# Mathiasb17/Nereus

Measured on AMD Instinct MI355X. Metric: particle-steps/sec, SESPH dam-break, higher is better.
Workload: dtype f32

## Files before the change

### nereus_amd/csrc/nrs_kernels_tiled.h

```cpp
#pragma once
#include "nrs_kernels_ref.h"
#include "nrs_kernels_slab.h"
#include <type_traits>

namespace nrs {

constexpr int HIT_CAP = 20;
constexpr uint32_t HIT_INDEX = (1u << 27) - 1;
constexpr int HIT_TAG_SHIFT = 27;

struct CutThresholds { float lenLtIr, r2LeH2; };

#ifndef FORCES_LISTS_MIN_WAVES
#define FORCES_LISTS_MIN_WAVES 7
#endif
#ifndef FORCES_PACKED_MIN_WAVES
#define FORCES_PACKED_MIN_WAVES 5
#endif
#ifndef FORCES_PACKED_MIN_WAVES_UNFUSED
#define FORCES_PACKED_MIN_WAVES_UNFUSED 4
#endif
NRS_DEV float bcast_lane(float v, int srcLane) { return __int_as_float(__builtin_amdgcn_readlane(__float_as_int(v), srcLane)); }
NRS_DEV double bcast_lane(double v, int srcLane)
{
    const long long b = __double_as_longlong(v);
    const int lo = __builtin_amdgcn_readlane((int)(b & 0xffffffffll), srcLane), hi = __builtin_amdgcn_readlane((int)(b >> 32), srcLane);
    return __longlong_as_double(((long long)hi << 32) | (long long)(unsigned int)lo);
}
#ifndef NRS_DBG_LDS_PAD
#define NRS_DBG_LDS_PAD 0
#endif
#ifndef NRS_DBG_LDS_PAD_F
#define NRS_DBG_LDS_PAD_F 0
#endif
#ifndef QP_WALK
#define QP_WALK 4
#endif
#ifndef QP_PRE
#define QP_PRE 2
#endif
constexpr int SCAN_CAP = 21;
NRS_DEV int mad24(int a, int b, int c)
{
    int d;
    asm("v_mad_i32_i24 %0, %1, %2, %3" : "=v"(d) : "v"(a), "v"(b), "v"(c));
    return d;
}
constexpr int SCAN_BATCH = 4;

struct HitCounts { int nf, nb; bool over; bool anyB; };
constexpr uint32_t GATHER_STRIDE = 2u;
template <typename R> struct PrePair { R prq, mrho; };

template <typename R> struct Sweep {
    typedef typename Vec4T<R>::type T4;
    static NRS_DEV T4 at32(const T4 *__restrict__ base, uint32_t idx)
    {
        const uint32_t off = idx * (uint32_t)sizeof(T4);
        return *reinterpret_cast<const T4 *>(reinterpret_cast<const char *>(base) + off);
    }

    template <bool HAS_B, int BFILT, int W, bool FWIDE = false>
    static NRS_DEV HitCounts scan(const Params<R> &P, const GridView<R> &G, const CutThresholds thr,
                                  const T4 *__restrict__ sPos, uint32_t self, V3<R> p, uint32_t (*lst)[W])
    {
        const I3 gp = calcGridPos<R>(P, p);
        const uint32_t mx = P.gridSize[0] - 1, my = P.gridSize[1] - 1, mz = P.gridSize[2] - 1;
        const uint32_t cx = grid_x<R>(P, gp.x);
        const uint32_t x0 = (cx - 1u) & mx, x2 = (cx + 1u) & mx;
        const bool contiguous = (cx >= 1u) && (cx + 1u <= mx);
        const float tF = FWIDE ? thr.r2LeH2 : thr.lenLtIr;
        const float tB = BFILT == 2 ? INFINITY : (BFILT == 1 ? thr.r2LeH2 : thr.lenLtIr);
        const uint32_t tid = threadIdx.x;
        int nf = 0, nb = 0;
        bool over = false, anyB = false;

        auto sweepFluid = [&](uint32_t a, uint32_t b, uint32_t m1, uint32_t m2, uint32_t tag0) {
            const uint32_t nT = run_ok<R>(G, a, b) ? b - a : 0u;
            for (uint32_t base = 0; base < nT; base += SCAN_BATCH) {
                T4 c[SCAN_BATCH];
#pragma unroll
                for (int u = 0; u < SCAN_BATCH; ++u) c[u] = at32(sPos, a + min(base + (uint32_t)u, nT - 1u));
#pragma unroll
                for (int u = 0; u < SCAN_BATCH; ++u) {
                    const uint32_t q = base + (uint32_t)u;
                    const uint32_t j = a + q;
                    const V3<R> d = p - xyz<R>(c[u]);
                    const bool hit = (q < nT) & (j != self) & (dot(d, d) < tF);
                    if (hit) {
                        uint32_t tag = tag0 + (((m1 != CELL_EMPTY) & (j >= m1)) ? 1u : 0u);
                        if ((m2 != CELL_EMPTY) & (j >= m2)) tag = tag0 + 2u;
                        if (nf + nb < HIT_CAP) lst[nf][tid] = j | (tag << HIT_TAG_SHIFT); else over = true;
                        ++nf;
                    }
                }
            }
        };

        for (int z = -1; z <= 1; z++) {
            const uint32_t cz = (uint32_t)(gp.z + z) & mz;
            const uint32_t plane = umul24(umul24(cz, P.gridSize[1]), P.gridSize[0]);
            uint32_t st[3][3], en[3][3], hrow[3];
            uint32_t bmask = 0;
#pragma unroll
            for (int y = 0; y < 3; ++y) {
                const uint32_t cy = (uint32_t)(gp.y + y - 1) & my;
                hrow[y] = plane + umul24(cy, P.gridSize[0]);
                const uint32_t h[3] = {hrow[y] + x0, hrow[y] + cx, hrow[y] + x2};
#pragma unroll
                for (int c = 0; c < 3; ++c) {
                    st[y][c] = G.cellStart[h[c]];
                    en[y][c] = G.cellEnd[h[c]];
                    if (HAS_B) bmask |= (G.bCellStart[h[c]] != CELL_EMPTY) ? (1u << (y * 3 + c)) : 0u;
                }
            }
#pragma unroll
            for (int y = 0; y < 3; ++y) {
                const uint32_t tag0 = (uint32_t)((z + 1) * 9 + y * 3);
                const uint32_t s0 = st[y][0], s1 = st[y][1], s2 = st[y][2];
                if (contiguous) {
                    uint32_t lo = (s0 != CELL_EMPTY) ? s0 : ((s1 != CELL_EMPTY) ? s1 : s2);
                    uint32_t hi = (s2 != CELL_EMPTY) ? en[y][2] : ((s1 != CELL_EMPTY) ? en[y][1] : en[y][0]);
                    if (lo == CELL_EMPTY) lo = hi = 0;
                    sweepFluid(lo, hi, s1, s2, tag0);
                } else {
#pragma unroll
                    for (int c = 0; c < 3; ++c)
                        if (st[y][c] != CELL_EMPTY) sweepFluid(st[y][c], en[y][c], CELL_EMPTY, CELL_EMPTY, tag0 + (uint32_t)c);
                }
            }
            if (HAS_B) {
                anyB = anyB || bmask != 0u;
                if (BFILT == 2) bmask = 0u;
                while (bmask) {
                    const int bit = __builtin_ctz(bmask);
                    bmask &= bmask - 1u;
                    const int y = bit / 3, c = bit - y * 3;
                    const uint32_t cy = (uint32_t)(gp.y + y - 1) & my;
                    const uint32_t hc = plane + umul24(cy, P.gridSize[0]) + (c == 0 ? x0 : (c == 1 ? cx : x2));
                    const uint32_t a = G.bCellStart[hc], nT = G.bCellEnd[hc] - a;
                    const uint32_t tag = (uint32_t)((z + 1) * 9 + bit);
                    for (uint32_t base = 0; base < nT; base += 4) {
                        T4 cb[4];
#pragma unroll
                        for (int u = 0; u < 4; ++u) cb[u] = G.sB[a + min(base + (uint32_t)u, nT - 1u)];
#pragma unroll
                        for (int u = 0; u < 4; ++u) {
                            const uint32_t q = base + (uint32_t)u;
                            const V3<R> d = p - xyz<R>(cb[u]);
                            if ((q < nT) & (dot(d, d) < tB)) {
                                if (nf + nb < HIT_CAP) lst[HIT_CAP - 1 - nb][tid] = (a + q) | (tag << HIT_TAG_SHIFT); else over = true;
                                ++nb;
                            }
                        }
                    }
                }
            }
        }
        HitCounts hc;
        const bool finite = (fabs(p.x) < (R)INFINITY) & (fabs(p.y) < (R)INFINITY) & (fabs(p.z) < (R)INFINITY);
        hc.nf = nf; hc.nb = nb; hc.over = over | !finite; hc.anyB = anyB;
        return hc;
    }

    static constexpr int QSLOTS = 16 / sizeof(qword_t);
    struct __attribute__((packed, aligned(sizeof(qword_t)))) Q2 { uint32_t v[4]; };
    static NRS_DEV Q2 ldq(const qword_t *__restrict__ qpos, uint32_t idx)
    {
        return *reinterpret_cast<const Q2 *>(reinterpret_cast<const char *>(qpos) + idx * (uint32_t)sizeof(qword_t));
    }
    template <int W>
    static NRS_DEV HitCounts scan_compact(const Params<R> &P, const GridView<R> &G, V3<R> p, uint32_t (*lst)[W])
    {
        const I3 gp = calcGridPos<R>(P, p);
        const uint32_t mx = P.gridSize[0] - 1, my = P.gridSize[1] - 1, mz = P.gridSize[2] - 1;
        const uint32_t cx = grid_x<R>(P, gp.x);
        const uint32_t x0 = (cx - 1u) & mx, x2 = (cx + 1u) & mx;
        const bool contiguous = (cx >= 1u) && (cx + 1u <= mx);
        float tx, ty, tz;
        quantize_t<R>(G.qc, p, tx, ty, tz);
        const bool far = !((fabsf(tx) < QP_FAR) & (fabsf(ty) < QP_FAR) & (fabsf(tz) < QP_FAR));
        const uint32_t Qi = pack_quanta(tx, ty, tz) | QP_GUARD;
        const uint32_t qT = G.qT;
        const qword_t *__restrict__ qpos = G.qpos;
        const uint32_t col = threadIdx.x * 4u, rowBytes = (uint32_t)W * 4u, capOff = col + (uint32_t)(SCAN_CAP + 1) * rowBytes;
        uint32_t cur = col;
        char *const lbase = reinterpret_cast<char *>(&lst[0][0]);

        auto test2 = [&](const Q2 &c, uint32_t aTag, uint32_t base, uint32_t nT) {
#pragma unroll
            for (int u = 0; u < QSLOTS; ++u) {
                if ((u & 1) == 0) cur = min(cur, capOff);
                const uint32_t t = Qi - c.v[u];
                const int dx = ((int)(t << 22)) >> 22, dy = ((int)(t << 11)) >> 22, dz = ((int)t) >> 22;
                const uint32_t d2 = (uint32_t)mad24(dz, dz, mad24(dy, dy, __mul24(dx, dx)));
                const uint32_t q = base + (uint32_t)u;
                const bool hit = (d2 < qT) & (q < nT);
                *reinterpret_cast<uint32_t *>(lbase + cur) = aTag + q;
                cur += hit ? rowBytes : 0u;
            }
        };
        auto sweepRun = [&](uint32_t aTag, uint32_t nT, uint32_t from) {
            for (uint32_t base = from; base < nT; base += QSLOTS) test2(ldq(qpos, (aTag & HIT_INDEX) + base), aTag, base, nT);
        };

        for (int z = -1; z <= 1; z++) {
            const uint32_t cz = (uint32_t)(gp.z + z) & mz;
            const uint32_t plane = umul24(umul24(cz, P.gridSize[1]), P.gridSize[0]);
            uint32_t st[3][3], en[3][3];
#pragma unroll
            for (int y = 0; y < 3; ++y) {
                const uint32_t cy = (uint32_t)(gp.y + y - 1) & my;
                const uint32_t hrow = plane + umul24(cy, P.gridSize[0]);
                const uint32_t h[3] = {hrow + x0, hrow + cx, hrow + x2};
#pragma unroll
                for (int c = 0; c < 3; ++c) {
                    const uint32_t off = h[c] * 4u;
                    st[y][c] = *reinterpret_cast<const uint32_t *>(reinterpret_cast<const char *>(G.cellStart) + off);
                    en[y][c] = *reinterpret_cast<const uint32_t *>(reinterpret_cast<const char *>(G.cellEnd) + off);
                }
            }
            if (contiguous) {
                uint32_t lo[3], nT[3];
#pragma unroll
                for (int y = 0; y < 3; ++y) {
                    const uint32_t s0 = st[y][0], s1 = st[y][1], s2 = st[y][2];
                    uint32_t a = (s0 != CELL_EMPTY) ? s0 : ((s1 != CELL_EMPTY) ? s1 : s2);
                    uint32_t b = (s2 != CELL_EMPTY) ? en[y][2] : ((s1 != CELL_EMPTY) ? en[y][1] : en[y][0]);
                    if (a == CELL_EMPTY) a = b = 0;
                    const bool ok = run_ok<R>(G, a, b);
                    lo[y] = ok ? a : 0u;
                    nT[y] = ok ? b - a : 0u;
                }
                Q2 c[3][QP_PRE];
#pragma unroll
                for (int y = 0; y < 3; ++y)
#pragma unroll
                    for (int k = 0; k < QP_PRE; ++k) c[y][k] = ldq(qpos, lo[y] + min((uint32_t)(QSLOTS * k), nT[y]));
#pragma unroll
                for (int y = 0; y < 3; ++y) {
                    const uint32_t aTag = lo[y] | ((uint32_t)((z + 1) * 9 + y * 3) << HIT_TAG_SHIFT);
#pragma unroll
                    for (int k = 0; k < QP_PRE; ++k)
                        if (k == 0 || nT[y] > (uint32_t)(QSLOTS * k))
                            test2(c[y][k], aTag, (uint32_t)(QSLOTS * k), nT[y]);
                    sweepRun(aTag, nT[y], (uint32_t)(QSLOTS * QP_PRE));
                }
            } else {
#pragma unroll
                for (int y = 0; y < 3; ++y)
#pragma unroll
                    for (int c = 0; c < 3; ++c)
                        if (st[y][c] != CELL_EMPTY && run_ok<R>(G, st[y][c], en[y][c]))
                            sweepRun(st[y][c] | ((uint32_t)((z + 1) * 9 + y * 3) << HIT_TAG_SHIFT), en[y][c] - st[y][c], 0u);
            }
        }
        const uint32_t nf = (cur - col) / rowBytes;
        HitCounts hc;
        hc.nf = (int)nf; hc.nb = 0; hc.over = far || nf > (uint32_t)SCAN_CAP; hc.anyB = false;
        return hc;
    }
};

struct HitMerge {
    const uint32_t *base;
    uint32_t stride;
    int nf, nb, kf, kb;
    uint32_t headF, headB;
    NRS_DEV HitMerge(const uint32_t *b, uint32_t st, HitCounts hc) : base(b), stride(st), nf(hc.nf), nb(hc.nb), kf(0), kb(0)
    {
        headF = nf > 0 ? base[0] : 0xffffffffu;
        headB = nb > 0 ? base[(uint32_t)(HIT_CAP - 1) * stride] : 0xffffffffu;
    }
    NRS_DEV int last_boundary() const { return kb - 1; }
    NRS_DEV bool next(uint32_t &index, bool &boundary, uint32_t &key)
    {
        if (kf >= nf && kb >= nb) return false;
        const uint32_t tf = headF >> HIT_TAG_SHIFT, tb = headB >> HIT_TAG_SHIFT;
        boundary = tb < tf;
        const uint32_t e = boundary ? headB : headF;
        if (boundary) {
            ++kb;
            headB = kb < nb ? base[(uint32_t)(HIT_CAP - 1 - kb) * stride] : 0xffffffffu;
        } else {
            ++kf;
            headF = kf < nf ? base[(uint32_t)kf * stride] : 0xffffffffu;
        }
        index = e & HIT_INDEX;
        key = (e >> HIT_TAG_SHIFT) * 2u + (boundary ? 1u : 0u);
        return true;
    }
};

template <typename R, int KSET, bool HAS_B, bool STRICT = false, bool BOUNDARY_BY_CELL = false>
NRS_DEV R density_from_hits(const Params<R> &P, const GridView<R> &G, const typename Vec4T<R>::type *__restrict__ sPos,
                            V3<R> p, const uint32_t *lbase, uint32_t lstride, HitCounts hc, uint32_t self = 0xffffffffu)
{
    const R ir = P.interactionRadius, kp = P.kpoly, pm = P.particleMass, rd = P.restDensity;
    R d = (R)0.0;
    d += pm * W_dens<R, KSET>(mk3<R>(0, 0, 0), ir, kp);
    if (BOUNDARY_BY_CELL) {
        const I3 gp = calcGridPos<R>(P, p);
        int k = 0;
        uint32_t head = hc.nf > 0 ? lbase[0] : 0xffffffffu;
        uint32_t c = 0;
        for (int z = -1; z <= 1; z++)
            for (int y = -1; y <= 1; y++)
                for (int x = -1; x <= 1; x++, c++) {
                    if ((head >> HIT_TAG_SHIFT) == c) {
                        R part = (R)0.0;
                        do {
                            const uint32_t j = head & HIT_INDEX;
                            const V3<R> r = p - xyz<R>(sPos[j]);
                            if (!STRICT || ((j != self) && (length(r) < ir))) part += (pm * W_dens<R, KSET>(r, ir, kp));
                            ++k;
                            head = k < hc.nf ? lbase[(uint32_t)k * lstride] : 0xffffffffu;
                        } while ((head >> HIT_TAG_SHIFT) == c);
                        d += part;
                    }
                    if (hc.anyB) {
                        const uint32_t h = calcGridHash<R>(P, gp.x + x, gp.y + y, gp.z + z);
                        const uint32_t sB = G.bCellStart[h];
                        if (sB != CELL_EMPTY) {
                            const uint32_t eB = G.bCellEnd[h];
                            R part = (R)0.0;
                            for (uint32_t j = sB; j < eB; ++j) {
                                const typename Vec4T<R>::type b = G.sB[j];
                                const V3<R> r = p - xyz<R>(b);
                                if (length(r) < ir) part += ((rd * b.w) * W_dens<R, KSET>(r, ir, kp));
                            }
                            d += part;
                        }
                    }
                }
        return d;
    }
    R part = (R)0.0;
    uint32_t prevKey = 0xffffffffu;
    HitMerge it(lbase, lstride, hc);
    uint32_t j, key;
    bool isB;
    while (it.next(j, isB, key)) {
        if (key != prevKey) { d += part; part = (R)0.0; prevKey = key; }
        if (HAS_B && isB) {
            const typename Vec4T<R>::type b = G.sB[j];
            const V3<R> r = p - xyz<R>(b);
            if (length(r) < ir) {
                const R psi = rd * b.w;
                part += (psi * W_dens<R, KSET>(r, ir, kp));
            }
        } else {
            const V3<R> r = p - xyz<R>(sPos[j]);
            if (!STRICT || ((j != self) && (length(r) < ir))) part += (pm * W_dens<R, KSET>(r, ir, kp));
        }
    }
    d += part;
    return d;
}

template <typename R, int KSET, bool STRICT, bool INRANGE = false>
NRS_DEV R density_from_superset(const Params<R> &P, const typename Vec4T<R>::type *__restrict__ sPos, V3<R> p, uint32_t (*lst)[BLOCK],
                                int &nf, float tKeep, uint32_t self)
{
    const uint32_t tid = threadIdx.x;
    const R ir = P.interactionRadius, kp = P.kpoly, pm = P.particleMass;
    const uint32_t mx = P.gridSize[0] - 1;
    const int gxi = (int)floor((p.x - P.worldOrigin[0]) / P.cellSize[0]);
    float yCell = 0.f;
    if constexpr (INRANGE) yCell = rcp_refined((float)P.cellSize[0]);
    R d = (R)0.0;
    d += pm * W_dens<R, KSET>(mk3<R>(0, 0, 0), ir, kp);
    R part = (R)0.0;
    uint32_t prevTag = 0xffffffffu;
    int w = 0;
    for (int k0 = 0; k0 < nf; k0 += QP_WALK) {
        uint32_t e[QP_WALK];
        V3<R> q[QP_WALK];
#pragma unroll
        for (int u = 0; u < QP_WALK; ++u) e[u] = lst[min(k0 + u, nf - 1)][tid];
#pragma unroll
        for (int u = 0; u < QP_WALK; ++u) q[u] = xyz<R>(sPos[e[u] & HIT_INDEX]);
#pragma unroll
        for (int u = 0; u < QP_WALK; ++u) {
            const V3<R> r = p - q[u];
            const uint32_t j = e[u] & HIT_INDEX;
            const float d2 = dot(r, r);
            if ((k0 + u < nf) && (d2 < tKeep) && (STRICT || j != self)) {
                int gxj;
                if constexpr (INRANGE) gxj = (int)floor(div_steps((float)(q[u].x - P.worldOrigin[0]), (float)P.cellSize[0], yCell));
                else gxj = (int)floor((q[u].x - P.worldOrigin[0]) / P.cellSize[0]);
                const uint32_t tag = (e[u] >> HIT_TAG_SHIFT) + (((uint32_t)(gxj - gxi) + 1u) & mx);
                lst[min(w, HIT_CAP - 1)][tid] = j | (tag << HIT_TAG_SHIFT);
                ++w;
                if (tag != prevTag) { d += part; part = (R)0.0; prevTag = tag; }
                if constexpr (INRANGE) {
                    const float len = d2 >= 0x1p-96f ? sqrt_inrange(d2) : sqrt_rn(d2);
                    if (!STRICT || ((j != self) && (len < ir))) {
                        const float r2 = len * len, h2 = ir * ir;
                        part += (pm * (r2 > h2 ? 0.0f : kp * cube_via_double<float>(h2 - r2)));
                    }
                } else {
                    if (!STRICT || ((j != self) && (length(r) < ir))) part += (pm * W_dens<R, KSET>(r, ir, kp));
                }
            }
        }
    }
    d += part;
    nf = w;
    return d;
}
template <typename R> NRS_DEV bool density_inrange_ok(const Params<R> &P, V3<R> p)
{
    if constexpr (!std::is_same<R, float>::value) return false;
    else {
        const float cs = P.cellSize[0], wo = fabsf(P.worldOrigin[0]);
        if (!(cs >= 0x1p-20f && cs <= 0x1p10f && wo <= 0x1p60f)) return false;
        if (wo >= 0x1p-60f) return true;
        return __all(fabsf(p.x - P.worldOrigin[0]) >= 4.0f * cs) != 0;
    }
}

template <typename R, int KSET> struct BoundaryTerms { V3<R> bound, pres, visc; };
template <typename R, int KSET>
NRS_DEV BoundaryTerms<R, KSET> boundary_terms(const Params<R> &P, V3<R> pos1, V3<R> vel1, R dens, R pres, typename Vec4T<R>::type bq)
{
    const R pm = P.particleMass, ir = P.interactionRadius;
    const R epsilon = (R)0.01;
    const R beta = P.beta, rd = P.restDensity;
    const R psi = (rd * bq.w);
    const V3<R> rij = pos1 - xyz<R>(bq);
    const V3<R> vij = vel1;
    R kernel;
    V3<R> grad;
    if (KSET == KS_MONAGHAN) {
        kernel = Wmonaghan<R>(rij, ir);
        grad = Wmonaghan_grad<R>(rij, ir);
    } else {
        kernel = Wdefault<R>(rij, ir, P.kpoly);
        grad = Wdefault_grad<R>(rij, ir, P.kpoly_grad);
    }
    BoundaryTerms<R, KSET> T;
    T.bound = (beta * psi * rij * kernel);
    T.pres = (-pm * psi * (pres / (dens * dens)) * grad);
    const R nuWall = (P.viscosity * ir * P.soundSpeed) / (dens * dens);
    const R approach = (R)fmax((double)dot(vij, rij), 0.0);
    const R normSq = dot(rij / length(rij), rij / length(rij)) + epsilon * ir * ir;
    const R friction = -nuWall * (approach / normSq);
    T.visc = (pm * psi * friction * grad);
    return T;
}

NRS_DEV f2 div2(f2 a, f2 b) { return pair2(a.x / b.x, a.y / b.y); }
struct InRange { float yVisc; uint32_t loBits, spanBits; bool constantsOk; };
NRS_DEV InRange in_range_setup(const Params<float> &P)
{
    InRange G;
    const float h = P.interactionRadius, h2 = h * h, kvd = fabsf(P.kvisc_denum);
    G.constantsOk = h >= 0x1p-10f && h <= 0x1p10f && kvd >= 0x1p-40f && kvd <= 0x1p40f;
    G.yVisc = rcp_refined(P.kvisc_denum);
    G.loBits = __float_as_uint(h2 * 0x1p-16f);
    G.spanBits = __float_as_uint(h2 * 2.0f) - G.loBits;
    return G;
}

struct PairTerms2 { V3x2 pres, visc, surf; };
template <bool SURF, bool INRANGE>
NRS_DEV PairTerms2 fluid_terms2_muller(const Params<float> &P, V3<float> pos1, V3<float> vel1, float own, float c0, float wAtDiameter, float diameter2,
                                       float4 pa, float4 pb, float4 va, float4 vb, PrePair<float> qa, PrePair<float> qb, const InRange &G, bool &bad)
{
    const float ir = P.interactionRadius, m2 = P.particleMass;
    float rxa = pos1.x - pa.x, rxb = pos1.x - pb.x, rya = pos1.y - pa.y, ryb = pos1.y - pb.y, rza = pos1.z - pa.z, rzb = pos1.z - pb.z;
    float vxa = vel1.x - va.x, vxb = vel1.x - vb.x, vya = vel1.y - va.y, vyb = vel1.y - vb.y, vza = vel1.z - va.z, vzb = vel1.z - vb.z;
    asm volatile("" : "+v"(rxa), "+v"(rxb), "+v"(rya), "+v"(ryb), "+v"(rza), "+v"(rzb));
    asm volatile("" : "+v"(vxa), "+v"(vxb), "+v"(vya), "+v"(vyb), "+v"(vza), "+v"(vzb));
    const V3x2 r = {pair2(rxa, rxb), pair2(rya, ryb), pair2(rza, rzb)};
    const V3x2 v = {pair2(vxa, vxb), pair2(vya, vyb), pair2(vza, vzb)};
    const f2 d2 = dot2(r, r);
    f2 len;
    if (INRANGE) {
        bad = bad || (__float_as_uint(d2.x) - G.loBits >= G.spanBits) || (__float_as_uint(d2.y) - G.loBits >= G.spanBits);
        len = sqrt_inrange2(d2);
    } else {
        len = pair2(sqrt_rn(d2.x), sqrt_rn(d2.y));
    }
    const f2 r2 = len * len;
    const float h2 = ir * ir;
    const bool outA = r2.x > h2, outB = r2.y > h2;
    const f2 hm = splat2(ir) - len;
    const f2 c = hm * hm;
    V3x2 gs;
    const f2 t3 = splat2(3.0f) * len;
    const f2 l3 = splat2(2.0f) * len * len * len;
    f2 cv;
    if (INRANGE) {
        const f2 y = rcp_refined2(len);
        gs.x = splat2(P.kpress_grad) * div_steps2(r.x, len, y) * c;
        gs.y = splat2(P.kpress_grad) * div_steps2(r.y, len, y) * c;
        gs.z = splat2(P.kpress_grad) * div_steps2(r.z, len, y) * c;
        cv = -div_steps2(t3, splat2(P.kvisc_denum), splat2(G.yVisc)) + splat2(2.0f / h2) - div_steps2(splat2(ir), l3, rcp_refined2(l3));
    } else {
        gs.x = splat2(P.kpress_grad) * div2(r.x, len) * c;
        gs.y = splat2(P.kpress_grad) * div2(r.y, len) * c;
        gs.z = splat2(P.kpress_grad) * div2(r.z, len) * c;
        cv = -div2(t3, splat2(P.kvisc_denum)) + splat2(2.0f / h2) - div2(splat2(ir), l3);
    }
    V3x2 gv = {splat2(P.kvisc_grad) * r.x * cv, splat2(P.kvisc_grad) * r.y * cv, splat2(P.kvisc_grad) * r.z * cv};
    const f2 hr = splat2(h2) - r2;
    f2 kern = splat2(P.kpoly) * pair2(cube_via_double<float>(hr.x), cube_via_double<float>(hr.y));
    if (outA) { gs.x.x = 0.f; gs.y.x = 0.f; gs.z.x = 0.f; gv.x.x = 0.f; gv.y.x = 0.f; gv.z.x = 0.f; kern.x = 0.f; }
    if (outB) { gs.x.y = 0.f; gs.y.y = 0.f; gs.z.y = 0.f; gv.x.y = 0.f; gv.y.y = 0.f; gv.z.y = 0.f; kern.y = 0.f; }
    PairTerms2 T;
    const f2 sp = splat2(m2) * (splat2(own) + pair2(qa.prq, qb.prq));
    T.pres.x = sp * gs.x; T.pres.y = sp * gs.y; T.pres.z = sp * gs.z;
    const f2 a = dot2(r, gv);
    const f2 b = d2 + splat2(0.01f * (ir * ir));
    const f2 q = div2(a, b);
    const f2 mr = pair2(qa.mrho, qb.mrho);
    T.visc.x = mr * v.x * q; T.visc.y = mr * v.y * q; T.visc.z = mr * v.z * q;
    if (SURF) {
        const f2 ks = pair2(d2.x > diameter2 ? kern.x : wAtDiameter, d2.y > diameter2 ? kern.y : wAtDiameter);
        const f2 z = splat2(0.f);
        T.surf.x = z - splat2(c0) * r.x * ks; T.surf.y = z - splat2(c0) * r.y * ks; T.surf.z = z - splat2(c0) * r.z * ks;
    }
    return T;
}

constexpr int LIST_BATCH = 4;
template <int NB = LIST_BATCH, typename GATHER, typename USE>
NRS_DEV void walk_fluid_batched(const uint32_t *col, uint32_t stride, int nf, GATHER &&gather, USE &&use)
{
    for (int k0 = 0; k0 < nf; k0 += NB) {
        uint32_t e[NB];
        decltype(gather(0u)) d[NB];
#pragma unroll
        for (int u = 0; u < NB; ++u) e[u] = col[(size_t)min(k0 + u, nf - 1) * stride];
#pragma unroll
        for (int u = 0; u < NB; ++u) d[u] = gather(e[u] & HIT_INDEX);
#pragma unroll
        for (int u = 0; u < NB; ++u)
            if (k0 + u < nf) use(e[u] & HIT_INDEX, e[u] >> HIT_TAG_SHIFT, d[u]);
    }
}

template <typename R, int KSET, bool SURF, bool HAS_B, bool STRICT = false, bool PAIRS = false, bool BOUNDARY_BY_CELL = false>
NRS_DEV ForceAcc<R> forces_from_hits(const Params<R> &P, const GridView<R> &G,
                                     const typename Vec4T<R>::type *__restrict__ sPos,
                                     const typename Vec4T<R>::type *__restrict__ sVel, const R *__restrict__ sDens,
                                     const R *__restrict__ sPres, V3<R> pos1, V3<R> vel1, R dens, R pres,
                                     const uint32_t *lbase, uint32_t lstride, HitCounts hc, uint32_t self = 0xffffffffu,
                                     const R *pre = nullptr, const typename Vec4T<R>::type *__restrict__ gpos = nullptr,
                                     const typename Vec4T<R>::type *__restrict__ gvel = nullptr, const uint32_t *__restrict__ lroot = nullptr,
                                     uint32_t lcol = 0u)
{
    ForceAcc<R> A;
    A.fpres = A.fvisc = A.fsurf = A.fbound = mk3<R>(0, 0, 0);
    const R pm = P.particleMass, m2 = P.particleMass, ir = P.interactionRadius, kp = P.kpoly;
    const R kappa = P.surfaceTension;
    const R kprg = P.kpress_grad, kvg = P.kvisc_grad, kvd = P.kvisc_denum;
    const R diameter = (R)(2.0 * P.particleRadius);
    const R diameter2 = diameter * diameter;
    const R rhoSqOwn = dens * dens;
    R wAtDiameter;
    if (KSET == KS_MONAGHAN) wAtDiameter = Wmonaghan<R>(mk3<R>(diameter, 0, 0), ir);
    else wAtDiameter = Wdefault<R>(mk3<R>(diameter, 0, 0), ir, kp);
    const R epsilon = (R)0.01;
    const R beta = P.beta, rd = P.restDensity;
    auto boundaryHit = [&](const BoundaryTerms<R, KSET> &T) {
        A.fbound = A.fbound + T.bound;
        A.fpres = A.fpres + T.pres;
        A.fvisc = A.fvisc - T.visc;
    };
    auto fluidHit = [&](uint32_t j) {
        V3<R> rij, vij;
        R pOverRhoSqNb, mOverRhoNb;
        if (PAIRS) {
            const typename Vec4T<R>::type a = gpos[GATHER_STRIDE * j], b = gvel[GATHER_STRIDE * j];
            rij = pos1 - xyz<R>(a);
            if (STRICT && ((j == self) || !(length(rij) < ir))) return;
            vij = vel1 - xyz<R>(b);
            pOverRhoSqNb = a.w; mOverRhoNb = b.w;
        } else {
            rij = pos1 - xyz<R>(sPos[j]);
            if (STRICT && ((j == self) || !(length(rij) < ir))) return;
            const R rhoNb = sDens[j];
            const R pNb = sPres[j];
            const R rhoSqNb = rhoNb * rhoNb;
            pOverRhoSqNb = pNb / rhoSqNb; mOverRhoNb = m2 / rhoNb;
            vij = vel1 - xyz<R>(sVel[j]);
        }
        V3<R> gradSpiky, gradVisc;
        R kernel;
        if (KSET == KS_MONAGHAN) {
            gradSpiky = Wmonaghan_grad<R>(rij, ir);
            gradVisc = gradSpiky;
            kernel = Wmonaghan<R>(rij, ir);
        } else {
            gradSpiky = Wpressure_grad<R>(rij, ir, kprg);
            gradVisc = Wviscosity_grad<R>(rij, ir, kvg, kvd);
            kernel = Wdefault<R>(rij, ir, kp);
        }
        A.fpres = A.fpres + (m2 * (pres / rhoSqOwn + pOverRhoSqNb) * gradSpiky);
        const R a = dot(rij, gradVisc);
        const R b = dot(rij, rij) + 0.01f * (ir * ir);
        A.fvisc = A.fvisc + (mOverRhoNb * vij * (a / b));
        if (SURF) {
            V3<R> ai = mk3<R>(0, 0, 0);
            const R r2 = dot(rij, rij);
            if (r2 > diameter2) ai = ai - (kappa / pm * pm * rij * kernel);
            else ai = ai - (kappa / pm * pm * rij * wAtDiameter);
            A.fsurf = A.fsurf + ai;
        }
    };
    if (BOUNDARY_BY_CELL) {
        const I3 gp = calcGridPos<R>(P, pos1);
        int k = 0;
        uint32_t head = hc.nf > 0 ? lbase[0] : 0xffffffffu;
        uint32_t c = 0;
        for (int z = -1; z <= 1; z++)
            for (int y = -1; y <= 1; y++)
                for (int x = -1; x <= 1; x++, c++) {
                    while ((head >> HIT_TAG_SHIFT) == c) {
                        fluidHit(head & HIT_INDEX);
                        ++k;
                        head = k < hc.nf ? lbase[(uint32_t)k * lstride] : 0xffffffffu;
                    }
                    if (hc.anyB) {
                        const uint32_t h = calcGridHash<R>(P, gp.x + x, gp.y + y, gp.z + z);
                        const uint32_t sB = G.bCellStart[h];
                        if (sB != CELL_EMPTY) {
                            const uint32_t eB = G.bCellEnd[h];
                            for (uint32_t j = sB; j < eB; ++j) boundaryHit(boundary_terms<R, KSET>(P, pos1, vel1, dens, pres, G.sB[j]));
                        }
                    }
                }
        return A;
    }
    if constexpr (!HAS_B && !STRICT && PAIRS && KSET == KS_MULLER && std::is_same<R, float>::value) {
        const int nf = hc.nf;
        const float own = pres / rhoSqOwn, c0 = kappa / pm * pm;
        auto walk = [&](auto inRange, const InRange &IG, bool &bad) {
            ForceAcc<R> S;
            S.fpres = S.fvisc = S.fsurf = S.fbound = mk3<R>(0, 0, 0);
            auto entry = [&](int k) { return lroot[(size_t)k * lstride + lcol]; };
            uint32_t e0 = nf > 0 ? entry(0) : 0u, e1 = nf > 1 ? entry(1) : e0;
            for (int k = 0; k < nf; k += 2) {
                const uint32_t j0 = e0 & HIT_INDEX, j1 = e1 & HIT_INDEX;
                const bool two = k + 1 < nf;
                const uint32_t n0 = k + 2 < nf ? entry(k + 2) : 0u;
                const uint32_t n1 = k + 3 < nf ? entry(k + 3) : n0;
                const float4 pa = gpos[GATHER_STRIDE * j0], pb = gpos[GATHER_STRIDE * j1], va = gvel[GATHER_STRIDE * j0], vb = gvel[GATHER_STRIDE * j1];
                const PairTerms2 T = fluid_terms2_muller<SURF, decltype(inRange)::value>(P, pos1, vel1, own, c0, wAtDiameter, diameter2, pa, pb, va, vb,
                                                                                        PrePair<float>{pa.w, va.w}, PrePair<float>{pb.w, vb.w}, IG, bad);
                S.fpres = S.fpres + mk3<R>(T.pres.x.x, T.pres.y.x, T.pres.z.x);
                S.fvisc = S.fvisc + mk3<R>(T.visc.x.x, T.visc.y.x, T.visc.z.x);
                if (SURF) S.fsurf = S.fsurf + mk3<R>(T.surf.x.x, T.surf.y.x, T.surf.z.x);
                if (two) {
                    S.fpres = S.fpres + mk3<R>(T.pres.x.y, T.pres.y.y, T.pres.z.y);
                    S.fvisc = S.fvisc + mk3<R>(T.visc.x.y, T.visc.y.y, T.visc.z.y);
                    if (SURF) S.fsurf = S.fsurf + mk3<R>(T.surf.x.y, T.surf.y.y, T.surf.z.y);
                }
                e0 = n0; e1 = n1;
            }
            return S;
        };
        const InRange IG = in_range_setup(P);
        const bool ownerOk = fminf(fminf(fabsf(pos1.x), fabsf(pos1.y)), fabsf(pos1.z)) >= 0x1p-66f;
        bool again = true;
        if (IG.constantsOk && __all(ownerOk)) {
            again = false;
            A = walk(std::true_type{}, IG, again);
        }
        if (again) A = walk(std::false_type{}, IG, again);
        return A;
    }
    HitMerge it(lbase, lstride, hc);
    uint32_t j, key;
    bool isB;
    while (it.next(j, isB, key)) {
        if (HAS_B && isB) {
            BoundaryTerms<R, KSET> T;
            if (pre) {
                const R *t = pre + (size_t)it.last_boundary() * 9;
                T.bound = mk3<R>(t[0], t[1], t[2]); T.pres = mk3<R>(t[3], t[4], t[5]); T.visc = mk3<R>(t[6], t[7], t[8]);
            } else {
                T = boundary_terms<R, KSET>(P, pos1, vel1, dens, pres, G.sB[j]);
            }
            boundaryHit(T);
        } else {
            fluidHit(j);
        }
    }
    return A;
}

NRS_DEV uint32_t xcd_tile(uint32_t b, uint32_t nb)
{
    const uint32_t per = nb >> 3;
    return (b < (per << 3)) ? (b & 7u) * per + (b >> 3) : b;
}

struct FastPair { float pr, invRho; };
struct HitBuffer {
    uint32_t *hits; uint32_t *counts; uint32_t stride;
    void *gpos = nullptr, *gvel = nullptr;
    const void *svel = nullptr;
    FastPair *fast = nullptr;
};
template <typename R> NRS_DEV typename Vec4T<R>::type own_sorted_velocity(const HitBuffer &hb, uint32_t i)
{
    return reinterpret_cast<const typename Vec4T<R>::type *>(hb.svel)[i];
}
template <typename R>
NRS_DEV void publish_gather_records(const Params<R> &P, const HitBuffer &hb, uint32_t i, V3<R> p, typename Vec4T<R>::type v, R d, R pr)
{
    typedef typename Vec4T<R>::type T4;
    reinterpret_cast<T4 *>(hb.gpos)[GATHER_STRIDE * i] = mk4<R>(p, pr / (d * d));
    reinterpret_cast<T4 *>(hb.gvel)[GATHER_STRIDE * i] = mk4<R>(xyz<R>(v), P.particleMass / d);
}
NRS_DEV uint32_t pack_counts(HitCounts hc)
{
    return (uint32_t)hc.nf | ((uint32_t)hc.nb << 8) | (hc.over ? 1u << 16 : 0u) | (hc.anyB ? 1u << 17 : 0u);
}
constexpr uint32_t COUNTS_UNSTAGED = 1u << 18;
NRS_DEV HitCounts unpack_counts(uint32_t c)
{
    HitCounts hc;
    hc.nf = (int)(c & 0xffu); hc.nb = (int)((c >> 8) & 0xffu); hc.over = ((c >> 16) & 1u) != 0u;
    hc.anyB = ((c >> 17) & 1u) != 0u;
    return hc;
}

static __global__ __launch_bounds__(BLOCK) void k_hit_stats(const uint32_t *__restrict__ counts, unsigned long long *__restrict__ out, uint32_t n)
{
    unsigned long long over = 0, sum = 0, mx = 0, unst = 0;
    for (uint32_t i = blockIdx.x * BLOCK + threadIdx.x; i < n; i += gridDim.x * BLOCK) {
        const uint32_t c = counts[i];
        const HitCounts hc = unpack_counts(c);
        unst += (c & COUNTS_UNSTAGED) ? 1ull : 0ull;
        if (hc.over) { ++over; continue; }
        const unsigned long long k = (unsigned long long)(hc.nf + hc.nb);
        sum += k;
        mx = k > mx ? k : mx;
    }
    for (int d = 32; d >= 1; d >>= 1) {
        over += __shfl_down(over, d);
        sum += __shfl_down(sum, d);
        unst += __shfl_down(unst, d);
        const unsigned long long o = __shfl_down(mx, d);
        mx = o > mx ? o : mx;
    }
    if ((threadIdx.x & 63u) == 0) {
        atomicAdd(&out[0], over);
        atomicAdd(&out[1], sum);
        atomicMax(&out[2], mx);
        atomicAdd(&out[3], unst);
    }
}

constexpr uint32_t COUNTS_DEFERRED = 1u << 19;

NRS_DEV bool cell_near_boundary(const WallList &wl, uint32_t h) { return ((wl.nearBits[h >> 5] >> (h & 31u)) & 1u) != 0u; }

static __global__ __launch_bounds__(BLOCK) void k_wall_compact(WallList wl, const uint32_t *__restrict__ tileOffset, const uint32_t *__restrict__ groupPrefix,
                                                                 uint32_t groupSize, uint32_t *__restrict__ list, uint32_t n)
{
    __shared__ uint32_t waveCnt[BLOCK / 64];
    const uint32_t i = blockIdx.x * BLOCK + threadIdx.x, lane = threadIdx.x & 63u, wave = threadIdx.x >> 6;
    const unsigned long long m = wl.mask[i >> 6];
    const bool take = ((m >> lane) & 1ull) != 0ull;
    if (lane == 0) waveCnt[wave] = (uint32_t)__popcll(m);
    __syncthreads();
    if (!take) return;
    uint32_t before = (uint32_t)__popcll(m & ((1ull << lane) - 1ull));
    for (uint32_t w = 0; w < wave; ++w) before += waveCnt[w];
    list[groupPrefix[blockIdx.x / groupSize] + tileOffset[blockIdx.x] + before] = i;
}

template <typename R, int KSET, bool HAS_B, bool SHARE, bool WIDE>
NRS_DEV void density_tiled_particle(const Params<R> &P, const GridView<R> &G, const CutThresholds thr,
                                    const typename Vec4T<R>::type *__restrict__ sPos, R *__restrict__ dens, R *__restrict__ pres,
                                    const HitBuffer &hb, uint32_t i, V3<R> p, uint32_t (*lst)[BLOCK], uint32_t countFlags = 0u)
{
    const uint32_t tid = threadIdx.x;
    constexpr int BF = SHARE ? (KSET == KS_MULLER ? 1 : 2) : 0;
    constexpr bool COMPACT = !HAS_B && SHARE;
    HitCounts hc;
    R d;
    if constexpr (COMPACT) {
        hc = Sweep<R>::template scan_compact<BLOCK>(P, G, p, lst);
        if (hc.over) d = density_of<R, KSET, HAS_B>(P, G, sPos, i);
        else {
            constexpr bool CAN = KSET == KS_MULLER && std::is_same<R, float>::value;
            const float tKeep = WIDE ? thr.r2LeH2 : thr.lenLtIr;
            if (CAN && density_inrange_ok<R>(P, p)) d = density_from_superset<R, KSET, WIDE, CAN>(P, sPos, p, lst, hc.nf, tKeep, i);
            else d = density_from_superset<R, KSET, WIDE>(P, sPos, p, lst, hc.nf, tKeep, i);
            if (hc.nf > HIT_CAP) { hc.over = true; d = density_of<R, KSET, HAS_B>(P, G, sPos, i); }
        }
    } else {
        hc = Sweep<R>::template scan<HAS_B, BF, BLOCK, WIDE>(P, G, thr, sPos, WIDE ? 0xffffffffu : i, p, lst);
        if (hc.over) d = density_of<R, KSET, HAS_B>(P, G, sPos, i);
        else d = density_from_hits<R, KSET, HAS_B, WIDE, (HAS_B && BF == 2)>(P, G, sPos, p, &lst[0][tid], BLOCK, hc, i);
    }
    dens[i] = d;
    if (pres) {
        const R pr = tait_pressure<R>(P, d);
        pres[i] = pr;
        if (SHARE && hb.gpos) publish_gather_records<R>(P, hb, i, p, own_sorted_velocity<R>(hb, i), d, pr);
        if (SHARE && hb.fast) {
            const float inv = __builtin_amdgcn_rcpf((float)d);
            FastPair z;
            z.pr = (float)pr * inv * inv; z.invRho = inv;
            hb.fast[i] = z;
        }
    }
    if (SHARE) {
        hb.counts[i] = pack_counts(hc) | countFlags;
        if (!hc.over) {
            for (int k = 0; k < hc.nf; ++k) hb.hits[(size_t)k * hb.stride + i] = lst[k][tid];
            for (int k = 0; k < hc.nb; ++k) hb.hits[(size_t)(HIT_CAP - 1 - k) * hb.stride + i] = lst[HIT_CAP - 1 - k][tid];
        }
    }
}

#ifndef DENSITY_DEFER_MIN_WAVES
#define DENSITY_DEFER_MIN_WAVES 6
#endif
template <typename R, int KSET, bool HAS_B, bool SHARE, bool WIDE = false, bool DEFER = false>
__global__ __launch_bounds__(BLOCK, (((DEFER || (!HAS_B && SHARE)) && sizeof(R) == 4) ? DENSITY_DEFER_MIN_WAVES : 1)) void k_density_tiled(Params<R> P, GridView<R> G, CutThresholds thr,
                                                         const typename Vec4T<R>::type *__restrict__ sPos,
                                                         R *__restrict__ dens, R *__restrict__ pres, HitBuffer hb,
                                                         uint32_t n, WallList wl, uint32_t wallBlocks)
{
    constexpr int LIST_ROWS = (SHARE && (DEFER || !HAS_B)) ? SCAN_CAP + 3 : HIT_CAP;
    __shared__ uint32_t lst[LIST_ROWS][BLOCK];
    uint32_t block = blockIdx.x, blocks = gridDim.x;
    if (DEFER) {
        if (block < wallBlocks) {
            const uint32_t count = *wl.count;
            for (uint32_t t = block * BLOCK + threadIdx.x; t < count; t += wallBlocks * BLOCK) {
                const uint32_t i = wl.list[t];
                const V3<R> p = xyz<R>(sPos[i]);
                if (!slab_active<R>(P, G, p.x)) {
                    dens[i] = (R)0;
                    if (pres) pres[i] = (R)0;
                    hb.counts[i] = COUNTS_DEFERRED;
                    continue;
                }
                density_tiled_particle<R, KSET, true, SHARE, WIDE>(P, G, thr, sPos, dens, pres, hb, i, p, lst, COUNTS_DEFERRED);
            }
            return;
        }
        block -= wallBlocks; blocks -= wallBlocks;
    }
    const uint32_t i = xcd_tile(block, blocks) * BLOCK + threadIdx.x;
    if (i >= n) return;
    if (DEFER && ((wl.mask[i >> 6] >> (i & 63u)) & 1ull)) return;
    const V3<R> p = xyz<R>(sPos[i]);
    if (!slab_active<R>(P, G, p.x)) {
        dens[i] = (R)0;
        if (pres) pres[i] = (R)0;
        if (SHARE) hb.counts[i] = 0u;
        return;
    }
    density_tiled_particle<R, KSET, HAS_B, SHARE, WIDE>(P, G, thr, sPos, dens, pres, hb, i, p, lst);
}

template <typename R> struct FusedOut {
    typedef typename Vec4T<R>::type T4;
    T4 *newPos, *newVel;
    uint32_t *hash, *index;
    const uint32_t *prevHash;
    uint32_t *tileMovers;
    uint8_t *slabFlags;
    uint32_t *slabBlockCounts;
    uint32_t slabBlocks;
    uint32_t *tileDead;
    SlabCfg slab;
};

template <typename R, int KSET, bool SURF, bool HAS_B, bool FUSE>
NRS_DEV void forces_epilogue(const Params<R> &P, typename Vec4T<R>::type p4, typename Vec4T<R>::type v4, V3<R> f,
                             typename Vec4T<R>::type *__restrict__ forces, const FusedOut<R> &fo, uint32_t i)
{
    if (forces) forces[i] = mk4<R>(f, (R)0);
    if (FUSE) {
        const R dt = P.timestep, m1 = P.particleMass;
        const V3<R> pos1 = xyz<R>(p4), vel1 = xyz<R>(v4);
        const V3<R> accel = dt * f / m1;
        const V3<R> v = vel1 + accel;
        const V3<R> pn = pos1 + dt * v;
        fo.newPos[i] = mk4<R>(pn, p4.w);
        fo.newVel[i] = mk4<R>(v, v4.w);
        const I3 g = calcGridPos<R>(P, pn);
        const uint32_t h = calcGridHash<R>(P, g.x, g.y, g.z);
        uint32_t key = h;
        if (fo.slabFlags) {
            const uint32_t f = slab_flags<R>(P, fo.slab, mk4<R>(pn, p4.w));
            fo.slabFlags[i] = (uint8_t)f;
            if (!(f & (1u << ST_STAY))) {
                key = 0xffffffffu;
                atomicAdd(&fo.tileDead[i / BLOCK], 1u);
            } else if (h != fo.prevHash[i]) {
                atomicAdd(&fo.tileMovers[i / BLOCK], 1u);
            }
            if (f & ~(1u << ST_STAY))
                for (int s = 1; s < ST_COUNT; ++s)
                    if ((f >> s) & 1u) atomicAdd(&fo.slabBlockCounts[(uint32_t)s * fo.slabBlocks + i / SLAB_TILE], 1u);
        } else if (fo.tileMovers && h != fo.prevHash[i]) {
            atomicAdd(&fo.tileMovers[i / BLOCK], 1u);
        }
        fo.hash[i] = key;
        fo.index[i] = i;
    }
}

template <typename R, int KSET, bool SURF, bool HAS_B, bool FUSE>
__global__ __launch_bounds__(BLOCK) void k_forces_tiled(Params<R> P, GridView<R> G, CutThresholds thr,
                                                        const typename Vec4T<R>::type *__restrict__ sPos,
                                                        const typename Vec4T<R>::type *__restrict__ sVel,
                                                        const R *__restrict__ sDens, const R *__restrict__ sPres,
                                                        typename Vec4T<R>::type *__restrict__ forces, FusedOut<R> fo,
                                                        uint32_t n)
{
    typedef typename Vec4T<R>::type T4;
    __shared__ uint32_t lst[HIT_CAP][BLOCK];
    const uint32_t i = xcd_tile(blockIdx.x, gridDim.x) * BLOCK + threadIdx.x;
    if (i >= n) return;
    const uint32_t tid = threadIdx.x;
    const T4 p4 = sPos[i];
    const T4 v4 = sVel[i];
    const V3<R> pos1 = xyz<R>(p4), vel1 = xyz<R>(v4);
    V3<R> f = mk3<R>(0, 0, 0);
    if (slab_active<R>(P, G, pos1.x)) {
        const R dens = sDens[i], pres = sPres[i];
        constexpr int BF = (KSET == KS_MULLER ? 1 : 2);
        const HitCounts hc = Sweep<R>::template scan<HAS_B, BF, BLOCK>(P, G, thr, sPos, i, pos1, lst);
        ForceAcc<R> A;
        if (hc.over) A = gather_forces<R, KSET, SURF, HAS_B>(P, G, i, pos1, vel1, dens, pres, sPos, sVel, sDens, sPres);
        else A = forces_from_hits<R, KSET, SURF, HAS_B, false, false, (HAS_B && BF == 2)>(P, G, sPos, sVel, sDens, sPres, pos1, vel1, dens, pres, &lst[0][tid], BLOCK, hc);
        f = sesph_total_force<R>(P, A, dens);
    }
    forces_epilogue<R, KSET, SURF, HAS_B, FUSE>(P, p4, v4, f, forces, fo, i);
}

template <typename R, int KSET, bool SURF, bool HAS_B, bool FUSE>
NRS_DEV void forces_lists_particle(const Params<R> &P, const GridView<R> &G, const HitBuffer &hb,
                                   const typename Vec4T<R>::type *__restrict__ sPos, const typename Vec4T<R>::type *__restrict__ sVel,
                                   const R *__restrict__ sDens, const R *__restrict__ sPres, typename Vec4T<R>::type *__restrict__ forces,
                                   const FusedOut<R> &fo, uint32_t i, typename Vec4T<R>::type p4, typename Vec4T<R>::type v4,
                                   bool active, HitCounts hc)
{
    const V3<R> pos1 = xyz<R>(p4), vel1 = xyz<R>(v4);
    V3<R> f = mk3<R>(0, 0, 0);
    if (active) {
        const R dens = sDens[i], pres = sPres[i];
        ForceAcc<R> A;
        if (hc.over) A = gather_forces<R, KSET, SURF, HAS_B>(P, G, i, pos1, vel1, dens, pres, sPos, sVel, sDens, sPres);
        else
            A = forces_from_hits<R, KSET, SURF, HAS_B, false, true, (HAS_B && KSET == KS_MONAGHAN)>(P, G, sPos, sVel, sDens, sPres, pos1, vel1, dens, pres, hb.hits + i, hb.stride,
                                                                                     hc, 0xffffffffu, nullptr, reinterpret_cast<const typename Vec4T<R>::type *>(hb.gpos),
                                                                                     reinterpret_cast<const typename Vec4T<R>::type *>(hb.gvel), hb.hits, i);
        f = sesph_total_force<R>(P, A, dens);
    }
    forces_epilogue<R, KSET, SURF, HAS_B, FUSE>(P, p4, v4, f, forces, fo, i);
}

template <typename R, int KSET, bool SURF, bool HAS_B, bool FUSE, bool DEFER = false>
__global__ __launch_bounds__(BLOCK, (sizeof(R) == 4 ? ((KSET == KS_MULLER && !HAS_B) ? (FUSE ? FORCES_PACKED_MIN_WAVES : FORCES_PACKED_MIN_WAVES_UNFUSED) : FORCES_LISTS_MIN_WAVES) : 1)) void k_forces_lists(Params<R> P, GridView<R> G, HitBuffer hb,
                                                        const typename Vec4T<R>::type *__restrict__ sPos,
                                                        const typename Vec4T<R>::type *__restrict__ sVel,
                                                        const R *__restrict__ sDens, const R *__restrict__ sPres,
                                                        typename Vec4T<R>::type *__restrict__ forces, FusedOut<R> fo,
                                                        uint32_t n, WallList wl, uint32_t wallBlocks)
{
    typedef typename Vec4T<R>::type T4;
    uint32_t block = blockIdx.x, blocks = gridDim.x;
    if (DEFER) {
        if (block < wallBlocks) {
            const uint32_t count = *wl.count;
            for (uint32_t t = block * BLOCK + threadIdx.x; t < count; t += wallBlocks * BLOCK) {
                const uint32_t i = wl.list[t];
                const T4 p4 = sPos[i];
                const bool active = slab_active<R>(P, G, p4.x);
                forces_lists_particle<R, KSET, SURF, true, FUSE>(P, G, hb, sPos, sVel, sDens, sPres, forces, fo, i, p4, sVel[i], active,
                                                                 unpack_counts(active ? hb.counts[i] : 0u));
            }
            return;
        }
        block -= wallBlocks; blocks -= wallBlocks;
    }
    const uint32_t i = xcd_tile(block, blocks) * BLOCK + threadIdx.x;
    if (i >= n) return;
    const uint32_t c = hb.counts[i];
    if (DEFER && (c & COUNTS_DEFERRED)) return;
    const T4 p4 = sPos[i];
    const bool active = slab_active<R>(P, G, p4.x);
    forces_lists_particle<R, KSET, SURF, HAS_B, FUSE>(P, G, hb, sPos, sVel, sDens, sPres, forces, fo, i, p4, sVel[i], active,
                                                      unpack_counts(active ? c : 0u));
}

template <typename R>
__global__ __launch_bounds__(BLOCK) void k_mark_near_boundary(Params<R> P, const uint32_t *__restrict__ bHash, uint32_t nb, uint32_t *__restrict__ nearBits)
{
    const uint32_t i = blockIdx.x * BLOCK + threadIdx.x;
    if (i >= nb) return;
    const uint32_t h = bHash[i];
    if (i && bHash[i - 1] == h) return;
    const uint32_t gx = P.gridSize[0], gy = P.gridSize[1];
    const int x = (int)((h & (gx - 1)) + P.numBodies), y = (int)((h / gx) & (gy - 1)), z = (int)(h / (gx * gy));
    for (int dz = -1; dz <= 1; ++dz)
        for (int dy = -1; dy <= 1; ++dy)
            for (int dx = -1; dx <= 1; ++dx) {
                const uint32_t c = calcGridHash<R>(P, x + dx, y + dy, z + dz);
                atomicOr(&nearBits[c >> 5], 1u << (c & 31u));
            }
}

static inline bool is_pow2(uint32_t v) { return v && !(v & (v - 1)); }

template <typename R> static inline CutThresholds make_thresholds(const Params<R> &P)
{
    CutThresholds t;
    const R ir = P.interactionRadius;
    {
        float T = (float)(ir * ir);
        auto ge = [&](float x) { return !((R)sqrtf(x) < ir); };
        while (ge(T) && T > 0.0f) T = nextafterf(T, 0.0f);
        while (!ge(T)) T = nextafterf(T, INFINITY);
        t.lenLtIr = T;
    }
    {
        const R h2 = ir * ir;
        float T = (float)h2;
        auto gt = [&](float x) { float l = sqrtf(x); R r2 = l * l; return r2 > h2; };
        while (gt(T) && T > 0.0f) T = nextafterf(T, 0.0f);
        while (!gt(T)) T = nextafterf(T, INFINITY);
        t.r2LeH2 = T;
    }
    return t;
}

static inline uint32_t wall_blocks(uint32_t interiorBlocks) { return std::min<uint32_t>(1024u, std::max<uint32_t>(1u, interiorBlocks / 16u)); }

template <typename R, int KSET, bool HAS_B>
static inline void launch_density_tiled(hipStream_t stream, const Params<R> &P, const GridView<R> &G, const HitBuffer *share,
                                        const typename Vec4T<R>::type *sPos, R *dens, R *pres, uint32_t n, const WallList *wall = nullptr)
{
    const CutThresholds thr = make_thresholds<R>(P);
    const dim3 g((n + BLOCK - 1) / BLOCK), b(BLOCK);
    const HitBuffer hb = share ? *share : HitBuffer{};
    constexpr unsigned pad = NRS_DBG_LDS_PAD;
    if (share) {
        if (HAS_B && wall) {
            const uint32_t wb = wall_blocks(g.x);
            hipLaunchKernelGGL((k_density_tiled<R, KSET, false, true, false, true>), dim3(g.x + wb), b, pad, stream, P, G, thr, sPos, dens, pres, hb, n,
                               *wall, wb);
        } else {
            hipLaunchKernelGGL((k_density_tiled<R, KSET, HAS_B, true>), g, b, pad, stream, P, G, thr, sPos, dens, pres, hb, n, WallList{}, 0u);
        }
    } else {
        hipLaunchKernelGGL((k_density_tiled<R, KSET, HAS_B, false>), g, b, 0, stream, P, G, thr, sPos, dens, pres, hb, n, WallList{}, 0u);
    }
}
template <typename R, int KSET, bool HAS_B>
static inline void launch_density_wide(hipStream_t stream, const Params<R> &P, const GridView<R> &G, const HitBuffer &hb,
                                       const typename Vec4T<R>::type *sPos, R *dens, uint32_t n, const WallList *wall = nullptr)
{
    const CutThresholds thr = make_thresholds<R>(P);
    const uint32_t g = (n + BLOCK - 1) / BLOCK;
    if (HAS_B && wall) {
        const uint32_t wb = wall_blocks(g);
        hipLaunchKernelGGL((k_density_tiled<R, KSET, false, true, true, true>), dim3(g + wb), dim3(BLOCK), 0, stream, P, G, thr, sPos, dens,
                           (R *)nullptr, hb, n, *wall, wb);
        return;
    }
    hipLaunchKernelGGL((k_density_tiled<R, KSET, HAS_B, true, true>), dim3(g), dim3(BLOCK), 0, stream, P, G, thr,
                       sPos, dens, (R *)nullptr, hb, n, WallList{}, 0u);
}
template <typename R, int KSET, bool SURF, bool HAS_B>
static inline void launch_forces_tiled(hipStream_t stream, const Params<R> &P, const GridView<R> &G, const HitBuffer *lists,
                                       const typename Vec4T<R>::type *sPos, const typename Vec4T<R>::type *sVel, const R *dens,
                                       const R *pres, typename Vec4T<R>::type *forces, const FusedOut<R> *fused, uint32_t n,
                                       const WallList *wall = nullptr)
{
    const FusedOut<R> fo = fused ? *fused : FusedOut<R>{};
    const dim3 g((n + BLOCK - 1) / BLOCK), b(BLOCK);
    constexpr unsigned padF = NRS_DBG_LDS_PAD_F;
    if (lists && HAS_B && wall) {
        const uint32_t wb = wall_blocks(g.x);
        const dim3 gd(g.x + wb);
        if (fused) hipLaunchKernelGGL((k_forces_lists<R, KSET, SURF, false, true, true>), gd, b, padF, stream, P, G, *lists, sPos, sVel, dens, pres, forces, fo, n, *wall, wb);
        else hipLaunchKernelGGL((k_forces_lists<R, KSET, SURF, false, false, true>), gd, b, 0, stream, P, G, *lists, sPos, sVel, dens, pres, forces, fo, n, *wall, wb);
    } else if (lists) {
        if (fused) hipLaunchKernelGGL((k_forces_lists<R, KSET, SURF, HAS_B, true>), g, b, padF, stream, P, G, *lists, sPos, sVel, dens, pres, forces, fo, n, WallList{}, 0u);
        else hipLaunchKernelGGL((k_forces_lists<R, KSET, SURF, HAS_B, false>), g, b, 0, stream, P, G, *lists, sPos, sVel, dens, pres, forces, fo, n, WallList{}, 0u);
    } else {
        const CutThresholds thr = make_thresholds<R>(P);
        if (fused) hipLaunchKernelGGL((k_forces_tiled<R, KSET, SURF, HAS_B, true>), g, b, 0, stream, P, G, thr, sPos, sVel, dens, pres, forces, fo, n);
        else hipLaunchKernelGGL((k_forces_tiled<R, KSET, SURF, HAS_B, false>), g, b, 0, stream, P, G, thr, sPos, sVel, dens, pres, forces, fo, n);
    }
}

}
```

Before: 5.178 billion.

## Stage neighbor pos/vel window in LDS for fluid-only Muller force gather

```diff
diff --git a/nereus_amd/csrc/nrs_kernels_tiled.h b/nereus_amd/csrc/nrs_kernels_tiled.h
--- a/nereus_amd/csrc/nrs_kernels_tiled.h
+++ b/nereus_amd/csrc/nrs_kernels_tiled.h
@@ -51,6 +51,14 @@
 struct HitCounts { int nf, nb; bool over; bool anyB; };
 constexpr uint32_t GATHER_STRIDE = 2u;
 template <typename R> struct PrePair { R prq, mrho; };
+constexpr uint32_t FORCE_WINDOW_HALO = 16u;
+constexpr uint32_t FORCE_WINDOW_SLOTS = BLOCK + 2u * FORCE_WINDOW_HALO;
+typedef float WindowVec __attribute__((ext_vector_type(4)));
+typedef const __attribute__((address_space(3))) WindowVec *WindowPtr;
+struct GatherWindow {
+    WindowPtr rec = nullptr; uint32_t lo = 0u, len = 0u;
+    NRS_DEV float4 load(uint32_t k) const { const WindowVec v = rec[k]; return make_float4(v.x, v.y, v.z, v.w); }
+};
 
 template <typename R> struct Sweep {
     typedef typename Vec4T<R>::type T4;
@@ -550,7 +558,7 @@
                                      const uint32_t *lbase, uint32_t lstride, HitCounts hc, uint32_t self = 0xffffffffu,
                                      const R *pre = nullptr, const typename Vec4T<R>::type *__restrict__ gpos = nullptr,
                                      const typename Vec4T<R>::type *__restrict__ gvel = nullptr, const uint32_t *__restrict__ lroot = nullptr,
-                                     uint32_t lcol = 0u)
+                                     uint32_t lcol = 0u, GatherWindow win = GatherWindow{})
 {
     ForceAcc<R> A;
     A.fpres = A.fvisc = A.fsurf = A.fbound = mk3<R>(0, 0, 0);
@@ -648,7 +656,13 @@
                 const bool two = k + 1 < nf;
                 const uint32_t n0 = k + 2 < nf ? entry(k + 2) : 0u;
                 const uint32_t n1 = k + 3 < nf ? entry(k + 3) : n0;
-                const float4 pa = gpos[GATHER_STRIDE * j0], pb = gpos[GATHER_STRIDE * j1], va = gvel[GATHER_STRIDE * j0], vb = gvel[GATHER_STRIDE * j1];
+                const uint32_t o0 = j0 - win.lo, o1 = j1 - win.lo, last = win.len - 1u;
+                float4 pa = win.load(GATHER_STRIDE * min(o0, last)), va = win.load(GATHER_STRIDE * min(o0, last) + 1u);
+                float4 pb = win.load(GATHER_STRIDE * min(o1, last)), vb = win.load(GATHER_STRIDE * min(o1, last) + 1u);
+                if (o0 > last) { pa = gpos[GATHER_STRIDE * j0]; va = gvel[GATHER_STRIDE * j0]; }
+                if (o1 > last) { pb = gpos[GATHER_STRIDE * j1]; vb = gvel[GATHER_STRIDE * j1]; }
+                asm volatile("" : "+v"(pa.x), "+v"(pa.y), "+v"(pa.z), "+v"(pa.w), "+v"(va.x), "+v"(va.y), "+v"(va.z), "+v"(va.w));
+                asm volatile("" : "+v"(pb.x), "+v"(pb.y), "+v"(pb.z), "+v"(pb.w), "+v"(vb.x), "+v"(vb.y), "+v"(vb.z), "+v"(vb.w));
                 const PairTerms2 T = fluid_terms2_muller<SURF, decltype(inRange)::value>(P, pos1, vel1, own, c0, wAtDiameter, diameter2, pa, pb, va, vb,
                                                                                         PrePair<float>{pa.w, va.w}, PrePair<float>{pb.w, vb.w}, IG, bad);
                 S.fpres = S.fpres + mk3<R>(T.pres.x.x, T.pres.y.x, T.pres.z.x);
@@ -948,7 +962,7 @@
                                    const typename Vec4T<R>::type *__restrict__ sPos, const typename Vec4T<R>::type *__restrict__ sVel,
                                    const R *__restrict__ sDens, const R *__restrict__ sPres, typename Vec4T<R>::type *__restrict__ forces,
                                    const FusedOut<R> &fo, uint32_t i, typename Vec4T<R>::type p4, typename Vec4T<R>::type v4,
-                                   bool active, HitCounts hc)
+                                   bool active, HitCounts hc, GatherWindow win = GatherWindow{})
 {
     const V3<R> pos1 = xyz<R>(p4), vel1 = xyz<R>(v4);
     V3<R> f = mk3<R>(0, 0, 0);
@@ -959,7 +973,7 @@
         else
             A = forces_from_hits<R, KSET, SURF, HAS_B, false, true, (HAS_B && KSET == KS_MONAGHAN)>(P, G, sPos, sVel, sDens, sPres, pos1, vel1, dens, pres, hb.hits + i, hb.stride,
                                                                                      hc, 0xffffffffu, nullptr, reinterpret_cast<const typename Vec4T<R>::type *>(hb.gpos),
-                                                                                     reinterpret_cast<const typename Vec4T<R>::type *>(hb.gvel), hb.hits, i);
+                                                                                     reinterpret_cast<const typename Vec4T<R>::type *>(hb.gvel), hb.hits, i, win);
         f = sesph_total_force<R>(P, A, dens);
     }
     forces_epilogue<R, KSET, SURF, HAS_B, FUSE>(P, p4, v4, f, forces, fo, i);
@@ -989,14 +1003,26 @@
         }
         block -= wallBlocks; blocks -= wallBlocks;
     }
-    const uint32_t i = xcd_tile(block, blocks) * BLOCK + threadIdx.x;
+    const uint32_t first = xcd_tile(block, blocks) * BLOCK, i = first + threadIdx.x;
+    if (first >= n) return;
+    GatherWindow win;
+    if constexpr (std::is_same<R, float>::value && KSET == KS_MULLER && !HAS_B) {
+        __shared__ float4 winRec[GATHER_STRIDE * FORCE_WINDOW_SLOTS];
+        const uint32_t end = min(n, first + BLOCK + FORCE_WINDOW_HALO);
+        win.lo = first > FORCE_WINDOW_HALO ? first - FORCE_WINDOW_HALO : 0u;
+        win.len = end - win.lo;
+        const float4 *src = reinterpret_cast<const float4 *>(hb.gpos) + GATHER_STRIDE * win.lo;
+        for (uint32_t t = threadIdx.x; t < GATHER_STRIDE * win.len; t += BLOCK) winRec[t] = src[t];
+        __syncthreads();
+        win.rec = reinterpret_cast<WindowPtr>(reinterpret_cast<uintptr_t>(&winRec[0]));
+    }
     if (i >= n) return;
     const uint32_t c = hb.counts[i];
     if (DEFER && (c & COUNTS_DEFERRED)) return;
     const T4 p4 = sPos[i];
     const bool active = slab_active<R>(P, G, p4.x);
     forces_lists_particle<R, KSET, SURF, HAS_B, FUSE>(P, G, hb, sPos, sVel, sDens, sPres, forces, fo, i, p4, sVel[i], active,
-                                                      unpack_counts(active ? c : 0u));
+                                                      unpack_counts(active ? c : 0u), win);
 }
 
 template <typename R>
```

Measured after the change: 5.250 billion, median of 6. +1.4%, better.
